# andimarafioti/faster-qwen3-tts

Measured on AMD Instinct MI355X. Metric: real-time factor (audio s / wall s), Qwen3-TTS-12Hz-0.6B voice-clone streaming chunk_size=8; p50 TTFA in ttfa_ms_p50, higher is better.
Workload: dtype bf16

## Files before the change

faster-qwen3-tts_amd/csrc/fq3_api.hip:

```cpp
#define FQ3_SKINNY_EXTERN
#include "fq3_ctx.h"
#include "sampler.cuh"
#include "sampler_wave.cuh"
#include "skinny_gemm.cuh"

#include <cstdio>
#include <cstdlib>
#include <cstring>
#include <map>
#include <string>
#include <type_traits>
#include <vector>

using namespace fq3;

static thread_local std::string g_err;
static int fail(int code, const std::string& m) { g_err = m; return code; }
int fq3_fail_(int code, const std::string& m) { return fail(code, m); }
#define HIPCHK(x) do { hipError_t e_ = (x); if (e_ != hipSuccess) return fail(FQ3_EHIP, std::string(#x) + ": " + hipGetErrorString(e_)); } while (0)

extern "C" const char* fq3_last_error(void) { return g_err.c_str(); }
extern "C" void fq3_set_error_(const char* msg) { g_err = msg ? msg : ""; }
extern "C" int fq3_abi_version(void) { return FQ3_ABI_VERSION; }

// ... 184 lines not shown
    const int Vm = std::max(t.vocab, p.vocab);
    const int G = cfg->num_code_groups;
    const int frames = cfg->max_frames > 0 ? cfg->max_frames : 4096;
    c->cfg.max_frames = frames;
    if ((r = dmalloc(c, &c->h, (size_t)Hm * c->esz))) return r;
    if ((r = dmalloc(c, &c->h2, (size_t)Hm * c->esz))) return r;
    if ((r = dmalloc(c, &c->qkv2, (size_t)qkvm * c->esz))) return r;
    if ((r = dmalloc(c, &c->attn_out, (size_t)qkvm * c->esz))) return r;
    if ((r = dmalloc(c, &c->attn_out2, (size_t)qkvm * c->esz))) return r;
    if ((r = dmalloc(c, &c->act2, (size_t)Im * c->esz))) return r;
    if ((r = dmalloc(c, &c->pred_x2, (size_t)p.hidden * c->esz))) return r;
    if ((r = dmalloc(c, &c->xin, (size_t)Hm * c->esz))) return r;
    if ((r = dmalloc(c, &c->tmp_hidden, (size_t)Hm * c->esz))) return r;
    if ((r = dmalloc(c, &c->qkv, (size_t)qkvm * c->esz))) return r;
    if ((r = dmalloc(c, &c->act, (size_t)Im * c->esz))) return r;
    if ((r = dmalloc(c, &c->logits, (size_t)Vm * c->esz))) return r;
    if ((r = dmalloc(c, &c->past_hidden, (size_t)t.hidden * c->esz))) return r;
    if ((r = dmalloc(c, &c->ph_hold, (size_t)t.hidden * c->esz))) return r;
    if ((r = dmalloc(c, &c->pred_in, (size_t)2 * t.hidden * c->esz))) return r;
    if ((r = dmalloc(c, &c->pred_next, (size_t)t.hidden * c->esz))) return r;
    if ((r = dmalloc(c, &c->pred_x, (size_t)p.hidden * c->esz))) return r;
    if ((r = dmalloc(c, &c->plogits, (size_t)(G - 1) * p.vocab * c->esz))) return r;
    const int maxkv = std::max(t.n_kv_heads, p.n_kv_heads);
    c->part_stride = (size_t)maxkv * kMaxWorkers * 4 * kPartStride;
    if ((r = dmalloc(c, (void**)&c->part, 2 * c->part_stride * sizeof(float)))) return r;
    if ((r = dmalloc(c, (void**)&c->rope_now, 2 * 64 * sizeof(float)))) return r;
    if ((r = dmalloc(c, (void**)&c->seen_api, kMaxVocab))) return r;
    if ((r = dmalloc(c, (void**)&c->st, sizeof(DecodeState)))) return r;
    if ((r = dmalloc(c, (void**)&c->seen, kMaxVocab))) return r;
    if ((r = dmalloc(c, (void**)&c->codes, (size_t)(frames + 1) * G * sizeof(int)))) return r;
    if ((r = dmalloc(c, (void**)&c->ids64, (size_t)64 * sizeof(int64_t)))) return r;
    if ((r = dmalloc(c, (void**)&c->d_pemb, (size_t)64 * sizeof(void*)))) return r;
    HIPCHK(hipStreamCreateWithFlags(&c->cap_stream, hipStreamNonBlocking));
    return FQ3_OK;
}

extern "C" int fq3_set_option(fq3_ctx* c, const char* key, int value) {
    if (!c || !key) return fail(FQ3_EINVAL, "null argument");
    const std::string k(key);
    if (k == "weight_nt") c->opt_nt = value;
    else if (k == "pred_m2") c->opt_m2 = value;
    else if (k == "pred_attn") c->opt_pred_attn = value;
    else if (k == "rows_per_wave_max") c->opt_rmax = value;
    else if (k == "prefill_mode") c->prefill_mode = value;
    else if (k == "flash_prefill") c->opt_flash_prefill = value;
    else if (k == "flash_small") c->opt_flash_small = value;
    else if (k == "swiglu_tile") c->opt_swiglu_tile = value;
    else if (k == "packed_weights") c->opt_packed = value;
    else if (k == "skinny_gemm") c->opt_no_skinny = !value;
    else return fail(FQ3_EINVAL, "unknown option: " + k);
    fq3_graph_reset(c);
    return FQ3_OK;
}

extern "C" int fq3_graph_reset(fq3_ctx* c) {
    if (!c) return fail(FQ3_EINVAL, "null ctx");
    if (c->exec) { (void)hipGraphExecDestroy(c->exec); c->exec = nullptr; }
    if (c->graph) { (void)hipGraphDestroy(c->graph); c->graph = nullptr; }
    return FQ3_OK;
}

namespace {
struct PackedEntry { void* p; int refs; int N, K; };
std::mutex g_packed_mu;
std::map<std::pair<const void*, int>, PackedEntry> g_packed;
}
// ... 30 lines not shown
}
static int packed_acquire_all(fq3_ctx* c) {
    if (c->cfg.dtype != FQ3_BF16) return FQ3_OK;
    auto take = [&](const void* W, int N, int K, int kind) -> int {
        const int r = fq3_packed_acquire_(W, N, K, kind);
        if (r == FQ3_OK) c->packed_refs.emplace_back(W, kind);
        return r == FQ3_EUNSUPPORTED ? FQ3_OK : r;
    };
    auto stack = [&](const std::vector<fq3_layer_weights>& L, const fq3_stack_dims& d) -> int {
        const int qd = d.n_heads * kHeadDim, kvd = d.n_kv_heads * kHeadDim;
        for (const fq3_layer_weights& l : L) {
            if (int r = take(l.qkv, qd + 2 * kvd, d.hidden, 0)) return r;
            if (int r = take(l.o, d.hidden, qd, 0)) return r;
            if (int r = take(l.gate_up, 2 * d.inter, d.hidden, 1)) return r;
            if (int r = take(l.gate_up, 2 * d.inter, d.hidden, 0)) return r;
            if (int r = take(l.down, d.hidden, d.inter, 0)) return r;
        }
        return FQ3_OK;
    };
    if (int r = stack(c->tl, c->cfg.talker)) return r;
    if (int r = stack(c->pl, c->cfg.predictor)) return r;
    for (const fq3_layer_weights& l : c->tl) if (int r = take(l.gate_up, 2 * c->cfg.talker.inter, c->cfg.talker.hidden, 2)) return r;
    if (int r = take(c->wt.codec_head, c->cfg.talker.vocab, c->cfg.talker.hidden, 0)) return r;
    for (const void* h : c->lmh) if (int r = take(h, c->cfg.predictor.vocab, c->cfg.predictor.hidden, 0)) return r;
    return FQ3_OK;
}

extern "C" int fq3_ctx_destroy(fq3_ctx* c) {
    if (!c) return FQ3_OK;
    (void)hipDeviceSynchronize();
    fq3_graph_reset(c);
    packed_release_all(c);
    if (c->cap_stream) (void)hipStreamDestroy(c->cap_stream);
    if (fq3_kv_pool* p = c->tk.pool) {
        (void)fq3_kv_release(c, 0);
        bool last;
        { std::lock_guard<std::mutex> lk(p->mu); last = --p->users == 0; }
        if (p->is_private && last) pool_free_(p);
    }
    for (void* p : c->allocs) (void)hipFree(p);
    delete c;
    return FQ3_OK;
}

extern "C" int fq3_bind_weights(fq3_ctx* c, const fq3_weight_table* w) {
    if (!c || !w) return fail(FQ3_EINVAL, "null argument");
    const int G = c->cfg.num_code_groups;
    if (!w->talker_layers || !w->predictor_layers || !w->codec_embedding || !w->codec_head || !w->talker_final_norm ||
        !w->predictor_final_norm || !w->predictor_embeddings || !w->lm_heads || !w->talker_cos || !w->talker_sin ||
        !w->pred_cos || !w->pred_sin)
        return fail(FQ3_EINVAL, "weight table has null entries");
    if (c->cfg.has_projection && !w->proj_w) return fail(FQ3_EINVAL, "has_projection set but proj_w is null");
    if (w->talker_rope_len < c->cfg.max_seq_len || w->pred_rope_len < G + 1)
        return fail(FQ3_EINVAL, "rope tables shorter than the caches");
    c->wt = *w;
    c->tl.assign(w->talker_layers, w->talker_layers + c->cfg.talker.n_layers);
    c->pl.assign(w->predictor_layers, w->predictor_layers + c->cfg.predictor.n_layers);
    c->pemb.assign(w->predictor_embeddings, w->predictor_embeddings + (G - 1));
    c->lmh.assign(w->lm_heads, w->lm_heads + (G - 1));
    for (auto& l : c->tl) if (!l.qkv || !l.o || !l.gate_up || !l.down || !l.input_norm || !l.post_norm || !l.q_norm || !l.k_norm)
        return fail(FQ3_EINVAL, "talker layer has null weights");
    for (auto& l : c->pl) if (!l.qkv || !l.o || !l.gate_up || !l.down || !l.input_norm || !l.post_norm || !l.q_norm || !l.k_norm)
        return fail(FQ3_EINVAL, "predictor layer has null weights");
    HIPCHK(hipMemcpy(c->d_pemb, c->pemb.data(), (G - 1) * sizeof(void*), hipMemcpyHostToDevice));
    (void)hipDeviceSynchronize();
    packed_release_all(c);
// ... 585 lines not shown
    tf->forced = forced; tf->decisions = decisions;
}

extern "C" int fq3_decode_begin(fq3_ctx* c, const fq3_decode_params* p, void* stream) {
    NEED_BOUND(c);
    if (!p || !p->past_hidden || !p->tts_pad_embed) return fail(FQ3_EINVAL, "null argument");
    if (p->trailing_len > 0 && !p->trailing_text) return fail(FQ3_EINVAL, "trailing_text");
    if (p->talker.do_sample && (!p->talker_noise || p->noise_frames <= 0)) return fail(FQ3_EINVAL, "talker sampling needs a noise ring");
    if (c->pred_sampling.do_sample && (!p->pred_noise || p->noise_frames <= 0)) return fail(FQ3_EINVAL, "predictor sampling needs a noise ring");
    if (p->talker.do_sample && !(p->talker.temperature > 0.f)) return fail(FQ3_EINVAL, "temperature must be > 0");
    if (p->max_new_tokens > c->cfg.max_frames) return fail(FQ3_EINVAL, "max_new_tokens exceeds the context's max_frames");
    if (p->prefill_len <= 0 || p->prefill_len > c->cfg.max_seq_len) return fail(FQ3_EINVAL, "prefill_len");
    if (p->first_token < 0 || p->first_token >= c->cfg.talker.vocab) return fail(FQ3_EINVAL, "first_token outside the codec vocabulary");
    if (p->gen_step < 0 || p->min_new_tokens < 0 || p->max_new_tokens < 0) return fail(FQ3_EINVAL, "negative counters");
    const bool wave = p->talker.top_p >= 1.0f;
    if (wave != c->talker_wave) { fq3_graph_reset(c); c->talker_wave = wave; }
    hipStream_t s = (hipStream_t)stream;
    if (int r = fq3_kv_ensure_(c, p->prefill_len + p->max_new_tokens + 1, s)) return r;
    DecodeState h{};
    h.token = p->first_token; h.frame = 0; h.pos = p->prefill_len; h.gen_step = p->gen_step; h.done = 0; h.text_open = 0;
    h.min_new = p->min_new_tokens; h.max_new = p->max_new_tokens; h.trailing_len = p->trailing_len;
    h.noise_frames = p->noise_frames > 0 ? p->noise_frames : 1;
    h.eos_id = c->cfg.codec_eos_token_id; h.max_seq = c->cfg.max_seq_len;
    h.n_pad = c->n_pad; h.rope_delta = c->rope_delta;
    h.sup_lo = c->cfg.talker.vocab - 1024 > 0 ? c->cfg.talker.vocab - 1024 : 0; h.sup_hi = c->cfg.talker.vocab;
    h.t_temperature = p->talker.temperature; h.t_top_k = p->talker.top_k; h.t_top_p = p->talker.top_p;
    h.t_do_sample = p->talker.do_sample; h.t_rep_penalty = p->talker.repetition_penalty;
    h.p_temperature = c->pred_sampling.temperature; h.p_top_k = c->pred_sampling.top_k; h.p_top_p = c->pred_sampling.top_p;
    h.p_do_sample = c->pred_sampling.do_sample;
    h.trailing_text = p->trailing_text; h.tts_pad = p->tts_pad_embed; h.talker_noise = p->talker_noise; h.pred_noise = p->pred_noise;
    hipLaunchKernelGGL(decode_arm_kernel, dim3(1), dim3(256), 0, s, c->st, h, c->seen, (int)kMaxVocab,
                       (uint32_t*)c->past_hidden, (const uint32_t*)p->past_hidden, (int)((size_t)c->cfg.talker.hidden * c->esz / 4));
    LAUNCH_CHECK();
    c->armed = true; c->tt_open = false; c->tt_session = false; c->tt_rows = 0; c->tt_cap = 0;
    c->begin_trailing = p->trailing_text; c->begin_trailing_len = p->trailing_len > 0 ? p->trailing_len : 0;
    return FQ3_OK;
}

__global__ void decode_cancel_kernel(DecodeState* st) { st->done = 1; }
extern "C" int fq3_decode_cancel(fq3_ctx* c, void* stream) {
    if (!c) return fail(FQ3_EINVAL, "null ctx");
    hipLaunchKernelGGL(decode_cancel_kernel, dim3(1), dim3(1), 0, (hipStream_t)stream, c->st);
    LAUNCH_CHECK();
    return FQ3_OK;
}

extern "C" int fq3_decode_set_forced(fq3_ctx* c, const int32_t* forced_codes, int32_t* decisions, void* stream) {
    NEED_BOUND(c);
    if (!c->tf) {
        if (!forced_codes && !decisions) return FQ3_OK;
        if (int r = dmalloc(c, (void**)&c->tf, sizeof(TeacherForcing))) return r;
        fq3_graph_reset(c);
    }
    hipLaunchKernelGGL(decode_set_forced_kernel, dim3(1), dim3(1), 0, (hipStream_t)stream, c->tf, forced_codes, decisions);
    LAUNCH_CHECK();
    return FQ3_OK;
}

template <typename T>
static int enqueue_frame_t(fq3_ctx* c, hipStream_t s) {
    const fq3_stack_dims& t = c->cfg.talker;
    const int G = c->cfg.num_code_groups, H = t.hidden;
    DecodeState* st = c->st;
    hipLaunchKernelGGL((frame_begin_kernel<T>), dim3(1), dim3(256), 0, s, st, (const T*)c->wt.codec_embedding,
                       (const T*)c->past_hidden, (T*)c->ph_hold, (T*)c->pred_in, c->codes, c->seen, H, G);
    if (int r = predictor_passes_t<T>(c, st, c->pred_in, nullptr, nullptr, nullptr, s)) return r;
// ... 16 lines not shown
    return c->cfg.dtype == FQ3_BF16 ? enqueue_frame_t<bf16_t>(c, s) : enqueue_frame_t<float>(c, s);
}

extern "C" int fq3_graph_capture(fq3_ctx* c, void* stream) {
    NEED_BOUND(c);
    if (c->exec) return FQ3_OK;
    (void)stream;
    hipStream_t cs = c->cap_stream;
    HIPCHK(hipStreamBeginCapture(cs, hipStreamCaptureModeRelaxed));
    int r = enqueue_frame(c, cs);
    hipGraph_t g = nullptr;
    hipError_t e = hipStreamEndCapture(cs, &g);
    if (r) { if (g) (void)hipGraphDestroy(g); return r; }
    if (e != hipSuccess) return fail(FQ3_EHIP, std::string("hipStreamEndCapture: ") + hipGetErrorString(e));
    c->graph = g;
    HIPCHK(hipGraphInstantiate(&c->exec, c->graph, nullptr, nullptr, 0));
    return FQ3_OK;
}

extern "C" int fq3_decode_frames(fq3_ctx* c, int n_frames, void* stream) {
    NEED_BOUND(c);
    hipStream_t s = (hipStream_t)stream;
    for (int i = 0; i < n_frames; ++i) {
        if (c->exec) { HIPCHK(hipGraphLaunch(c->exec, s)); }
        else if (int r = enqueue_frame(c, s)) return r;
    }
    LAUNCH_CHECK();
    return FQ3_OK;
}

extern "C" int fq3_decode_poll(fq3_ctx* c, int* n_frames_total, int* done, void* stream) {
    if (!c) return fail(FQ3_EINVAL, "null ctx");
    hipStream_t s = (hipStream_t)stream;
    DecodeState h;
    HIPCHK(hipMemcpyAsync(&h, c->st, sizeof h, hipMemcpyDeviceToHost, s));
    HIPCHK(hipStreamSynchronize(s));
    if (n_frames_total) *n_frames_total = h.frame;
    if (done) *done = h.done == 2 ? 2 : (h.done || h.token == h.eos_id);
    return FQ3_OK;
}

__global__ void codes_to_i64_kernel(const int* src, int64_t* dst, int n) {
    const int i = blockIdx.x * blockDim.x + threadIdx.x;
    if (i < n) dst[i] = src[i];
}

extern "C" int fq3_decode_codes(fq3_ctx* c, int from, int count, int64_t* out, void* stream) {
    if (!c || !out) return fail(FQ3_EINVAL, "null argument");
    if (from < 0 || count < 0 || from + count > c->cfg.max_frames) return fail(FQ3_EINVAL, "range");
    const int G = c->cfg.num_code_groups, n = count * G;
    if (n == 0) return FQ3_OK;
    hipLaunchKernelGGL(codes_to_i64_kernel, dim3((n + 255) / 256), dim3(256), 0, (hipStream_t)stream,
                       c->codes + (size_t)from * G, out, n);
    LAUNCH_CHECK();
    return FQ3_OK;
}
```

faster-qwen3-tts_amd/csrc/fq3_ctx.h:

```cpp
#pragma once
#include "../../include/fq3hip.h"
#include "decode_kernels.cuh"
#include <hip/hip_runtime.h>
#include <mutex>
#include <string>
#include <utility>
#include <vector>

struct fq3_kv_pool {
    int dtype = 0, esz = 2, n_layers = 0, n_kv = 0, n_blocks = 0;
    size_t blk_elems = 0;
    std::vector<void*> k, v;
    std::vector<int> free_list;
    std::mutex mu;
    int in_use_high = 0;
    int users = 0;
    bool is_private = false;
};

struct StackBufs {
    std::vector<void*> k, v;
    int max_seq = 0, workers = 1;
    fq3_kv_pool* pool = nullptr;
    int* d_table = nullptr;
    std::vector<int> blocks;
    int max_blocks = 0;
};

struct fq3_ctx {
    fq3_config cfg{};
    int esz = 2;
    std::vector<fq3_layer_weights> tl, pl;
    fq3_weight_table wt{};
    std::vector<const void*> pemb, lmh;
    const void** d_pemb = nullptr;
    bool bound = false;
    StackBufs tk, pk;
    void *h = nullptr, *xin = nullptr, *qkv = nullptr, *act = nullptr, *logits = nullptr, *past_hidden = nullptr;
    void *pred_in = nullptr, *pred_x = nullptr, *pred_next = nullptr, *plogits = nullptr, *tmp_hidden = nullptr;
    void *attn_out = nullptr, *attn_out2 = nullptr;
    void *h2 = nullptr, *qkv2 = nullptr, *act2 = nullptr, *pred_x2 = nullptr;
    size_t part_stride = 0;
    float* part = nullptr;
    float* rope_now = nullptr;
    unsigned char* seen_api = nullptr;
    fq3::DecodeState* st = nullptr;
    fq3::TeacherForcing* tf = nullptr;
    unsigned char* seen = nullptr;
    int* codes = nullptr;
    int64_t* ids64 = nullptr;
    int n_pad = 0, rope_delta = 0;
    int opt_nt = 1;
    int opt_m2 = 1;
    int opt_pred_attn = 1;
    int opt_rmax = 2;
    int opt_flash_prefill = 1;
    int opt_flash_small = 1;
    int opt_swiglu_tile = 1;
    int opt_packed = 1;
    std::vector<std::pair<const void*, int>> packed_refs;
    int opt_no_skinny = 0;
    int prefill_mode = 0;
    bool talker_wave = true;
    fq3_sampling pred_sampling{0.9f, 50, 1.0f, 1, 1.0f};
    hipGraph_t graph = nullptr;
    hipGraphExec_t exec = nullptr;
    hipStream_t cap_stream = nullptr;
    std::vector<void*> allocs;
    fq3_prompt_weights pw{};
    bool pw_bound = false;
    void *pw_x = nullptr, *pw_h = nullptr;
    int pw_cap = 0;
    void* ph_hold = nullptr;
    void *tt_tab = nullptr, *tt_x = nullptr, *tt_h = nullptr;
    int tt_alloc = 0;
    int tt_cap = 0, tt_rows = 0;
    bool tt_open = false, tt_session = false;
    bool armed = false;
    const void* begin_trailing = nullptr; int begin_trailing_len = 0;
    void *pf_x = nullptr, *pf_xn = nullptr, *pf_qkv = nullptr, *pf_att = nullptr, *pf_gu = nullptr, *pf_act = nullptr, *pf_ws = nullptr;
};


const void* fq3_packed_find_(const void* W, int kind);
int fq3_packed_acquire_(const void* W, int N, int K, int kind);
void fq3_packed_release_(const void* W, int kind);

int fq3_fail_(int code, const std::string& m);
int fq3_kv_ensure_(fq3_ctx* c, int n_pos, hipStream_t s);
int fq3_prefill_reserve_(fq3_ctx* c);
int fq3_prefill_mfma_(fq3_ctx* c, const void* embeds, int L, int n_pad, void* out_logits, void* out_hidden, hipStream_t s);
int fq3_prefill_batch_mfma_(fq3_ctx* const* cs, int n, const void* const* embeds, const int* L, const int* n_pad, void* const* out_logits,
                            void* const* out_hidden, hipStream_t s);
int fq3_codec_head_launch_(fq3_ctx* c, const void* hidden, void* out_logits, hipStream_t s);
int fq3_dmalloc_(fq3_ctx* c, void** p, size_t bytes);
void fq3_text_project_launch_(fq3_ctx* c, const int64_t* ids, int n, void* x, void* h, void* out, hipStream_t s);
```

faster-qwen3-tts_amd/fq3hip/_lib.py:

```python
from __future__ import annotations

import ctypes as C
import os

import torch

_HERE = os.path.dirname(os.path.abspath(__file__))
LIB_PATH = os.path.join(os.path.dirname(_HERE), "lib", "libfq3hip.so")

FQ3_BF16, FQ3_F32, FQ3_BF16X2 = 0, 1, 2
FQ3_OK, FQ3_EINVAL, FQ3_EHIP, FQ3_ESTATE, FQ3_ETOOLONG, FQ3_EUNSUPPORTED, FQ3_ENOMEM = 0, -1, -2, -3, -4, -5, -6

vp = C.c_void_p
i32 = C.c_int32


class StackDims(C.Structure):
    _fields_ = [("hidden", i32), ("inter", i32), ("n_layers", i32), ("n_heads", i32), ("n_kv_heads", i32),
                ("head_dim", i32), ("vocab", i32), ("rms_eps", C.c_float)]


class Config(C.Structure):
    _fields_ = [("dtype", i32), ("talker", StackDims), ("predictor", StackDims), ("num_code_groups", i32),
                ("max_seq_len", i32), ("codec_eos_token_id", i32), ("has_projection", i32), ("max_frames", i32)]
# ... 54 lines not shown
    "fq3_ctx_create": (C.c_int, [C.POINTER(Config), C.POINTER(vp)]),
    "fq3_ctx_destroy": (C.c_int, [vp]),
    "fq3_kv_pool_create": (C.c_int, [C.POINTER(Config), C.c_int, C.POINTER(vp)]),
    "fq3_kv_pool_destroy": (C.c_int, [vp]),
    "fq3_kv_pool_stats": (C.c_int, [vp, C.POINTER(C.c_int), C.POINTER(C.c_int), C.POINTER(C.c_int), C.POINTER(C.c_int64)]),
    "fq3_ctx_create_pooled": (C.c_int, [C.POINTER(Config), vp, C.POINTER(vp)]),
    "fq3_kv_reserve": (C.c_int, [vp, C.c_int, vp]),
    "fq3_kv_release": (C.c_int, [vp, C.c_int]),
    "fq3_kv_blocks": (C.c_int, [vp]),
    "fq3_bind_weights": (C.c_int, [vp, C.POINTER(WeightTable)]),
    "fq3_set_option": (C.c_int, [vp, C.c_char_p, C.c_int]),
    "fq3_kv_import": (C.c_int, [vp, C.c_int, vp, vp, C.c_int, vp]),
    "fq3_kv_export": (C.c_int, [vp, C.c_int, vp, vp, C.c_int, vp]),
    "fq3_kv_adopt": (C.c_int, [vp, vp, C.c_int, vp]),
    "fq3_set_generation_state": (C.c_int, [vp, C.c_int, C.c_int]),
    "fq3_talker_step": (C.c_int, [vp, vp, C.c_int, vp, vp]),
    "fq3_prefill": (C.c_int, [vp, vp, C.c_int, C.c_int, vp, vp, vp]),
    "fq3_prefill_reserve": (C.c_int, [vp]),
    "fq3_prefill_batch": (C.c_int, [C.POINTER(vp), C.c_int, C.POINTER(vp), C.POINTER(C.c_int), C.POINTER(C.c_int), C.POINTER(vp),
                                    C.POINTER(vp), vp]),
    "fq3_set_prefill_mode": (C.c_int, [vp, C.c_int]),
    "fq3_codec_head": (C.c_int, [vp, vp, vp, vp]),
    "fq3_set_predictor_sampling": (C.c_int, [vp, C.POINTER(Sampling)]),
    "fq3_predictor_loop": (C.c_int, [vp, vp, vp, vp, vp, vp]),
    "fq3_sample": (C.c_int, [vp, vp, C.c_int, C.POINTER(Sampling), vp, C.c_int, C.c_int, C.c_int, C.c_int,
                             C.c_int, vp, vp, vp]),
    "fq3_apply_repetition_penalty": (C.c_int, [vp, vp, C.c_int, vp, C.c_int, C.c_float, vp]),
    "fq3_decode_begin": (C.c_int, [vp, C.POINTER(DecodeParams), vp]),
    "fq3_decode_cancel": (C.c_int, [vp, vp]),
    "fq3_decode_set_forced": (C.c_int, [vp, vp, vp, vp]),
    "fq3_decode_frames": (C.c_int, [vp, C.c_int, vp]),
    "fq3_decode_poll": (C.c_int, [vp, C.POINTER(C.c_int), C.POINTER(C.c_int), vp]),
    "fq3_decode_codes": (C.c_int, [vp, C.c_int, C.c_int, vp, vp]),
    "fq3_graph_capture": (C.c_int, [vp, vp]),
    "fq3_graph_reset": (C.c_int, [vp]),
    "fq3_bind_prompt_weights": (C.c_int, [vp, C.POINTER(PromptWeights)]),
    "fq3_text_project": (C.c_int, [vp, vp, C.c_int, vp, vp]),
    "fq3_decode_text_open": (C.c_int, [vp, C.c_int, vp]),
    "fq3_decode_text_append": (C.c_int, [vp, vp, C.c_int, C.c_int, vp]),
    "fq3_decode_text_rows": (C.c_int, [vp, C.POINTER(C.c_int), C.POINTER(C.c_int)]),
    "fq3_decode_text_read": (C.c_int, [vp, C.c_int, C.c_int, vp, vp]),
    "fq3_prompt_rows": (C.c_int, [vp, vp, C.c_int, vp, C.c_int, vp, C.c_int, vp, vp, vp]),
    "fq3_batch_create": (C.c_int, [C.POINTER(vp), C.c_int, C.POINTER(vp)]),
    "fq3_batch_destroy": (C.c_int, [vp]),
    "fq3_batch_size": (C.c_int, [vp]),
    "fq3_batch_frames": (C.c_int, [vp, C.c_int, vp]),
    "fq3_batch_graph_capture": (C.c_int, [vp, vp]),
    "fq3_batch_graph_reset": (C.c_int, [vp]),
    "fq3_batch_set_option": (C.c_int, [vp, C.c_char_p, C.c_int]),
    "fq3_batch_set_group_streams": (C.c_int, [vp, C.POINTER(vp), C.c_int]),
    "fq3_batch_poll_async": (C.c_int, [vp, C.c_int, vp]),
    "fq3_batch_poll_wait": (C.c_int, [vp, C.c_int, C.POINTER(C.c_int), C.POINTER(C.c_int)]),
    "fq3_batch_text_append": (C.c_int, [vp, C.c_int, C.POINTER(C.c_int32), C.POINTER(C.c_int32), C.POINTER(C.c_int32), vp, vp]),
    "fq3_codec_create": (C.c_int, [C.POINTER(CodecConfig), C.POINTER(vp)]),
    "fq3_codec_destroy": (C.c_int, [vp]),
    "fq3_codec_set_option": (C.c_int, [vp, C.c_char_p, C.c_int]),
    "fq3_codec_bind": (C.c_int, [vp, C.c_char_p, vp, C.c_int64]),
    "fq3_codec_finalize": (C.c_int, [vp, vp]),
    "fq3_codec_num_samples": (C.c_int64, [vp, C.c_int]),
    "fq3_codec_decode": (C.c_int, [vp, vp, C.c_int, vp, vp]),
    "fq3_codec_decode_tail": (C.c_int, [vp, vp, C.c_int, C.c_int64, vp, vp]),
    "fq3_codec_decode_batch": (C.c_int, [vp, vp, C.c_int, C.c_int, C.c_int64, vp, vp]),
    "fq3_codec_prefix_create": (C.c_int, [vp, vp, C.c_int, C.POINTER(vp), vp]),
    "fq3_codec_prefix_destroy": (C.c_int, [vp]),
    "fq3_codec_prefix_frames": (C.c_int, [vp]),
    "fq3_codec_decode_batch_prefix": (C.c_int, [vp, C.POINTER(vp), vp, C.c_int, C.c_int, C.c_int64, vp, vp]),
# ... 45 lines not shown
```

faster-qwen3-tts_amd/fq3hip/engine.py:

```python
from __future__ import annotations

import ctypes as C
import threading
from typing import Dict, Optional

import torch

from . import _lib as L
from .config import TTSConfig, StackConfig

Weights = Dict[str, torch.Tensor]
_CAPTURE_LOCK = threading.Lock()


def _ptr(t: Optional[torch.Tensor]) -> Optional[int]:
    return None if t is None else t.data_ptr()


def rope_tables(head_dim: int, theta: float, n_pos: int, dtype: torch.dtype):
    inv = 1.0 / (theta ** (torch.arange(0, head_dim, 2, dtype=torch.float) / head_dim))
    ang = torch.arange(n_pos, dtype=torch.float32)[:, None] * inv[None, :]
    return ang.cos().to(dtype).float().contiguous(), ang.sin().to(dtype).float().contiguous()


# ... 343 lines not shown
        tl = trailing_text.shape[-2] if trailing_text is not None and trailing_text.numel() else 0
        if tl:
            self._chk(trailing_text, tl * H, "trailing_text")
        p = L.DecodeParams()
        p.talker = L.Sampling(float(temperature), int(top_k), float(top_p), int(bool(do_sample)), float(repetition_penalty))
        p.min_new_tokens, p.max_new_tokens = int(min_new_tokens), int(max_new_tokens)
        p.prefill_len, p.gen_step, p.first_token = int(prefill_len), int(gen_step), int(first_token)
        p.past_hidden, p.trailing_text, p.trailing_len = past_hidden.data_ptr(), _ptr(trailing_text) if tl else None, tl
        p.tts_pad_embed = tts_pad_embed.data_ptr()
        p.talker_noise, p.pred_noise, p.noise_frames = _ptr(talker_noise), _ptr(pred_noise), int(noise_frames)
        self._loop_keep = (past_hidden, trailing_text, tts_pad_embed, talker_noise, pred_noise)
        L.check(self.lib.fq3_decode_begin(self.ctx, C.byref(p), self._stream()))

    def graph_capture(self):
        with _CAPTURE_LOCK:
            L.check(self.lib.fq3_graph_capture(self.ctx, self._stream()))

    def graph_reset(self):
        L.check(self.lib.fq3_graph_reset(self.ctx))

    def decode_frames(self, n: int):
        L.check(self.lib.fq3_decode_frames(self.ctx, int(n), self._stream()))

    def decode_poll(self):
        n, d = C.c_int(0), C.c_int(0)
        L.check(self.lib.fq3_decode_poll(self.ctx, C.byref(n), C.byref(d), self._stream()))
        return n.value, bool(d.value)

    def decode_poll_state(self):
        n, d = C.c_int(0), C.c_int(0)
        L.check(self.lib.fq3_decode_poll(self.ctx, C.byref(n), C.byref(d), self._stream()))
        return n.value, int(d.value)

    def decode_text_open(self, capacity_rows: int):
        L.check(self.lib.fq3_decode_text_open(self.ctx, int(capacity_rows), self._stream()))

    def decode_text_append(self, ids, final: bool = False):
        if isinstance(ids, torch.Tensor):
            t = ids.reshape(-1).to(device=self.device, dtype=torch.long).contiguous()
        else:
            t = torch.tensor([int(i) for i in ids], dtype=torch.long, device=self.device)
        n = int(t.numel())
        L.check(self.lib.fq3_decode_text_append(self.ctx, t.data_ptr() if n else None, n, int(bool(final)), self._stream()))
        self._text_ids_keep = t

    def decode_text_rows(self):
        n, c = C.c_int(0), C.c_int(0)
        L.check(self.lib.fq3_decode_text_rows(self.ctx, C.byref(n), C.byref(c)))
        return n.value, bool(c.value)

    def decode_text_read(self, start: int = 0, count: Optional[int] = None) -> torch.Tensor:
        if count is None:
            count = self.decode_text_rows()[0] - int(start)
        out = self.new(int(count), self.cfg.talker.hidden_size)
        L.check(self.lib.fq3_decode_text_read(self.ctx, int(start), int(count), out.data_ptr(), self._stream()))
        return out

    def decode_codes(self, start: int, count: int) -> torch.Tensor:
        out = torch.empty(count, self.cfg.num_code_groups, dtype=torch.long, device=self.device)
        if count:
            L.check(self.lib.fq3_decode_codes(self.ctx, int(start), int(count), out.data_ptr(), self._stream()))
        return out

    def close(self):
        if getattr(self, "ctx", None) and self.ctx.value:
            self.lib.fq3_ctx_destroy(self.ctx)
# ... 87 lines not shown
```

faster-qwen3-tts_amd/fq3hip/generate.py:

```python
from __future__ import annotations

import time
from typing import Optional, Tuple

import torch

from .predictor_graph import PredictorGraph
from .talker_graph import TalkerGraph

NOISE_RING = 64


def _refill(engine, talker_noise, pred_noise):
    if talker_noise is not None:
        talker_noise.exponential_(1)
    if pred_noise is not None:
        pred_noise.exponential_(1)


def _n_pad_of(attention_mask) -> int:
    if attention_mask is None:
        return 0
    known = noted_n_pad(attention_mask)
    return known if known is not None else int((attention_mask[0] == 0).sum())


def noted_n_pad(attention_mask):
    note = getattr(attention_mask, "fq3_n_pad", None)
    if not (isinstance(note, tuple) and len(note) == 2):
        return None
    if note[1] is None:
        return int(note[0])
    if attention_mask.is_inference() or note[1] != attention_mask._version:
        return None
    return int(note[0])


def _prefill_first_token(eng, talker_input_embeds, attention_mask, config, min_new_tokens, temperature, top_k, top_p, do_sample):
    dt, dev = eng.dtype, eng.device
    eos_id = config.codec_eos_token_id
    V = config.vocab_size
    n_pad = _n_pad_of(attention_mask)
    x = talker_input_embeds[0].to(device=dev, dtype=dt).contiguous()
# ... 58 lines not shown
    max_frames = min(int(max_new_tokens), eng.max_frames)
    eng.decode_begin(first_token=int(token), prefill_len=prefill_len, gen_step=gen_step, past_hidden=hidden,
                     trailing_text=tth, tts_pad_embed=tpe, temperature=temperature, top_k=top_k, top_p=top_p,
                     do_sample=do_sample, repetition_penalty=repetition_penalty, min_new_tokens=min_new_tokens,
                     max_new_tokens=max_frames, talker_noise=tn, pred_noise=pn, noise_frames=NOISE_RING)
    if use_graph:
        eng.graph_capture()
    else:
        eng.graph_reset()
    return eng, tn, pn, max_frames


def _prefill_and_arm(talker, talker_input_embeds, attention_mask, trailing_text_hiddens, tts_pad_embed, config,
                     predictor_graph, talker_graph, max_new_tokens, min_new_tokens, temperature, top_k, top_p,
                     do_sample, repetition_penalty, use_graph):
    token, hidden, n_rows, n_pad = _prefill_first_token(talker_graph.engine, talker_input_embeds, attention_mask, config,
                                                        min_new_tokens, temperature, top_k, top_p, do_sample)
    return _arm_decode(talker, config, token, hidden, n_rows, attention_mask, trailing_text_hiddens, tts_pad_embed, predictor_graph,
                       talker_graph, max_new_tokens, min_new_tokens, temperature, top_k, top_p, do_sample, repetition_penalty,
                       use_graph, n_pad=n_pad)


def run_frames(eng, tn, pn, issued: int, count: int):
    while count > 0:
        if issued % NOISE_RING == 0:
            _refill(eng, tn, pn)
        k = min(count, NOISE_RING - issued % NOISE_RING)
        eng.decode_frames(k)
        issued += k
        count -= k
    return issued


@torch.inference_mode()
def fast_generate(talker, talker_input_embeds: torch.Tensor, attention_mask: torch.Tensor,
                  trailing_text_hiddens: torch.Tensor, tts_pad_embed: torch.Tensor, config,
                  predictor_graph: PredictorGraph, talker_graph: TalkerGraph, max_new_tokens: int = 2048,
                  min_new_tokens: int = 2, temperature: float = 0.9, top_k: int = 50, top_p: float = 1.0,
                  do_sample: bool = True, repetition_penalty: float = 1.05,
                  subtalker_dosample: Optional[bool] = None, subtalker_top_k: Optional[int] = None,
                  subtalker_top_p: Optional[float] = None, subtalker_temperature: Optional[float] = None,
                  parity_mode: bool = False, poll_every: int = 8) -> Tuple[Optional[torch.Tensor], dict]:
    t_start = time.time()
    eng, tn, pn, max_frames = _prefill_and_arm(
        talker, talker_input_embeds, attention_mask, trailing_text_hiddens, tts_pad_embed, config, predictor_graph,
        talker_graph, max_new_tokens, min_new_tokens, temperature, top_k, top_p, do_sample, repetition_penalty,
        use_graph=not parity_mode)
    torch.cuda.current_stream(eng.device).synchronize()
    t_prefill = time.time() - t_start
    t_decode_start = time.time()
    issued, n, done = 0, 0, False
    while not done and issued < max_frames:
        issued = run_frames(eng, tn, pn, issued, min(poll_every, max_frames - issued))
        n, done = eng.decode_poll()
    codes = eng.decode_codes(0, n) if n > 0 else None
    torch.cuda.current_stream(eng.device).synchronize()
    t_decode = time.time() - t_decode_start
    timing = {
        "prefill_ms": t_prefill * 1000,
        "decode_s": t_decode,
        "steps": n,
        "ms_per_step": (t_decode / n * 1000) if n > 0 else 0,
        "steps_per_s": (n / t_decode) if t_decode > 0 else 0,
    }
    return codes, timing
```

faster-qwen3-tts_amd/fq3hip/streaming.py:

```python
from __future__ import annotations

import time
from typing import Generator, Tuple

import torch

from .generate import _prefill_and_arm, run_frames
from .predictor_graph import PredictorGraph
from .talker_graph import TalkerGraph


@torch.inference_mode()
def fast_generate_streaming(talker, talker_input_embeds: torch.Tensor, attention_mask: torch.Tensor,
                            trailing_text_hiddens: torch.Tensor, tts_pad_embed: torch.Tensor, config,
                            predictor_graph: PredictorGraph, talker_graph: TalkerGraph, max_new_tokens: int = 2048,
                            min_new_tokens: int = 2, temperature: float = 0.9, top_k: int = 50, top_p: float = 1.0,
                            do_sample: bool = True, repetition_penalty: float = 1.05, chunk_size: int = 12,
                            use_graph: bool = True) -> Generator[Tuple[torch.Tensor, dict], None, None]:
    t_start = time.time()
    eng, tn, pn, max_frames = _prefill_and_arm(
        talker, talker_input_embeds, attention_mask, trailing_text_hiddens, tts_pad_embed, config, predictor_graph,
        talker_graph, max_new_tokens, min_new_tokens, temperature, top_k, top_p, do_sample, repetition_penalty,
        use_graph=use_graph)
    torch.cuda.current_stream(eng.device).synchronize()
    t_prefill = time.time() - t_start
    issued, emitted, chunk_count, done = 0, 0, 0, False
    chunk_start = time.time()
    issued = run_frames(eng, tn, pn, issued, min(chunk_size, max_frames))
    while True:
        n, done = eng.decode_poll()
        new = n - emitted
        if new <= 0:
            break
        chunk = eng.decode_codes(emitted, new)
        ready = torch.cuda.Event()
        ready.record(torch.cuda.current_stream(eng.device))
        emitted = n
        is_final = new < chunk_size
        more = (not done) and (not is_final) and issued < max_frames
        if more:
            issued = run_frames(eng, tn, pn, issued, min(chunk_size, max_frames - issued))
        yield chunk, {
            "chunk_index": chunk_count,
            "chunk_steps": new,
            "prefill_ms": t_prefill * 1000 if chunk_count == 0 else 0,
            "decode_ms": (time.time() - chunk_start) * 1000,
            "total_steps_so_far": emitted,
            "is_final": is_final,
            "codes_ready_event": ready,
        }
        chunk_count += 1
        chunk_start = time.time()
        if not more:
            break


def parity_generate_streaming(talker, talker_input_embeds, attention_mask, trailing_text_hiddens, tts_pad_embed, config,
                              max_new_tokens: int = 2048, min_new_tokens: int = 2, temperature: float = 0.9,
                              top_k: int = 50, top_p: float = 1.0, do_sample: bool = True,
                              repetition_penalty: float = 1.05, chunk_size: int = 12, predictor_graph=None,
                              talker_graph=None):
    if predictor_graph is None or talker_graph is None:
        raise ValueError("parity_generate_streaming needs the graph objects of the HIP context")
    return fast_generate_streaming(talker, talker_input_embeds, attention_mask, trailing_text_hiddens, tts_pad_embed,
                                   config, predictor_graph, talker_graph, max_new_tokens=max_new_tokens,
                                   min_new_tokens=min_new_tokens, temperature=temperature, top_k=top_k, top_p=top_p,
                                   do_sample=do_sample, repetition_penalty=repetition_penalty, chunk_size=chunk_size,
                                   use_graph=False)
```

include/fq3hip.h:

```cpp
#ifndef FQ3HIP_H
#define FQ3HIP_H

#include <stdint.h>

#ifdef __cplusplus
extern "C" {
#endif

#define FQ3_ABI_VERSION 5

enum { FQ3_BF16 = 0, FQ3_F32 = 1,
       FQ3_BF16X2 = 2 };
enum { FQ3_OK = 0, FQ3_EINVAL = -1, FQ3_EHIP = -2, FQ3_ESTATE = -3, FQ3_ETOOLONG = -4, FQ3_EUNSUPPORTED = -5, FQ3_ENOMEM = -6 };

typedef struct fq3_stack_dims {
    int32_t hidden, inter, n_layers, n_heads, n_kv_heads, head_dim, vocab;
    float rms_eps;
} fq3_stack_dims;

typedef struct fq3_config {
    int32_t dtype;
    fq3_stack_dims talker;
    fq3_stack_dims predictor;
    int32_t num_code_groups;
// ... 85 lines not shown
                       void* out_logits, void* stream);


int fq3_sample(fq3_ctx* ctx, const void* logits, int V, const fq3_sampling* s, const int64_t* history,
               int n_hist, int sup_lo, int sup_hi, int keep_id, int suppress_eos, const void* noise,
               int64_t* out_token, void* stream);

int fq3_apply_repetition_penalty(fq3_ctx* ctx, void* logits, int V, const int64_t* history, int n_hist, float penalty,
                                 void* stream);


typedef struct fq3_decode_params {
    fq3_sampling talker;
    int32_t min_new_tokens;
    int32_t max_new_tokens;
    int32_t prefill_len;
    int32_t gen_step;
    int32_t first_token;
    const void* past_hidden;
    const void* trailing_text;
    int32_t trailing_len;
    const void* tts_pad_embed;
    const void* talker_noise;
    const void* pred_noise;
    int32_t noise_frames;
} fq3_decode_params;

int fq3_decode_begin(fq3_ctx* ctx, const fq3_decode_params* p, void* stream);
int fq3_decode_cancel(fq3_ctx* ctx, void* stream);
int fq3_decode_set_forced(fq3_ctx* ctx, const int32_t* forced_codes, int32_t* decisions, void* stream);
int fq3_decode_frames(fq3_ctx* ctx, int n_frames, void* stream);
int fq3_decode_poll(fq3_ctx* ctx, int* n_frames_total, int* done, void* stream);
int fq3_decode_codes(fq3_ctx* ctx, int from, int count, int64_t* out_codes_dev, void* stream);
int fq3_graph_capture(fq3_ctx* ctx, void* stream);
int fq3_graph_reset(fq3_ctx* ctx);

typedef struct fq3_prompt_weights {
    const void* text_embedding;
    const void* fc1_w;
    const void* fc1_b;
    const void* fc2_w;
    const void* fc2_b;
    int32_t text_vocab, text_hidden;
} fq3_prompt_weights;
int fq3_bind_prompt_weights(fq3_ctx* ctx, const fq3_prompt_weights* w);
int fq3_text_project(fq3_ctx* ctx, const int64_t* ids, int n, void* out, void* stream);
int fq3_prompt_rows(fq3_ctx* ctx, const void* text_rows, int n_text, const int32_t* prog, int n_rows,
                    const int64_t* ref_codes, int n_ref, const void* spk_embed, void* out, void* stream);

int fq3_decode_text_open(fq3_ctx* ctx, int capacity_rows, void* stream);
int fq3_decode_text_append(fq3_ctx* ctx, const int64_t* ids, int n, int final, void* stream);
int fq3_decode_text_rows(const fq3_ctx* ctx, int* n_rows, int* closed);
int fq3_decode_text_read(fq3_ctx* ctx, int from, int count, void* out, void* stream);

typedef struct fq3_batch fq3_batch;
int fq3_batch_create(fq3_ctx* const* lanes, int n_lanes, fq3_batch** out);
int fq3_batch_destroy(fq3_batch* b);
int fq3_batch_size(const fq3_batch* b);
int fq3_batch_frames(fq3_batch* b, int n_frames, void* stream);
int fq3_batch_graph_capture(fq3_batch* b, void* stream);
int fq3_batch_graph_reset(fq3_batch* b);
int fq3_batch_poll_async(fq3_batch* b, int slot, void* stream);
int fq3_batch_poll_wait(fq3_batch* b, int slot, int* n_frames_total, int* done);
int fq3_batch_text_append(fq3_batch* b, int n_items, const int32_t* lane, const int32_t* count, const int32_t* final_,
                          const int64_t* ids, void* stream);
int fq3_batch_set_option(fq3_batch* b, const char* key, int value);
// ... 55 lines not shown
```

Before: 37.15.

## Queue async decode polls and run frames ahead of chunk marker

Adds an asynchronous poll API: a small kernel snapshots decode state and copies the chunk's codes, then writes the status into pinned host memory tracked by an event per slot. The streaming and non-streaming loops now issue a few frames beyond each chunk marker before waiting on the poll, so the GPU stays busy while the host reads status and yields chunks. The goal is to remove the idle GPU bubble caused by a blocking stream synchronize and a separate codes copy each chunk. The cost is extra frames of speculative work after EOS and more complex slot and event bookkeeping.

```diff
diff --git a/faster-qwen3-tts_amd/csrc/fq3_api.hip b/faster-qwen3-tts_amd/csrc/fq3_api.hip
--- a/faster-qwen3-tts_amd/csrc/fq3_api.hip
+++ b/faster-qwen3-tts_amd/csrc/fq3_api.hip
@@ -240,6 +240,9 @@
     if ((r = dmalloc(c, (void**)&c->ids64, (size_t)64 * sizeof(int64_t)))) return r;
     if ((r = dmalloc(c, (void**)&c->d_pemb, (size_t)64 * sizeof(void*)))) return r;
     HIPCHK(hipStreamCreateWithFlags(&c->cap_stream, hipStreamNonBlocking));
+    if ((r = dmalloc(c, (void**)&c->poll_dev, (size_t)kDecodePollSlots * 2 * sizeof(int)))) return r;
+    HIPCHK(hipHostMalloc((void**)&c->poll_host, (size_t)kDecodePollSlots * 2 * sizeof(int) + sizeof(DecodeState), hipHostMallocDefault));
+    for (int i = 0; i < kDecodePollSlots; ++i) HIPCHK(hipEventCreateWithFlags(&c->poll_ev[i], hipEventDisableTiming));
     return FQ3_OK;
 }
 
@@ -336,6 +339,8 @@
     fq3_graph_reset(c);
     packed_release_all(c);
     if (c->cap_stream) (void)hipStreamDestroy(c->cap_stream);
+    for (hipEvent_t e : c->poll_ev) if (e) (void)hipEventDestroy(e);
+    if (c->poll_host) (void)hipHostFree(c->poll_host);
     if (fq3_kv_pool* p = c->tk.pool) {
         (void)fq3_kv_release(c, 0);
         bool last;
@@ -987,6 +992,7 @@
     hipLaunchKernelGGL(decode_arm_kernel, dim3(1), dim3(256), 0, s, c->st, h, c->seen, (int)kMaxVocab,
                        (uint32_t*)c->past_hidden, (const uint32_t*)p->past_hidden, (int)((size_t)c->cfg.talker.hidden * c->esz / 4));
     LAUNCH_CHECK();
+    for (bool& a : c->poll_armed) a = false;
     c->armed = true; c->tt_open = false; c->tt_session = false; c->tt_rows = 0; c->tt_cap = 0;
     c->begin_trailing = p->trailing_text; c->begin_trailing_len = p->trailing_len > 0 ? p->trailing_len : 0;
     return FQ3_OK;
@@ -1069,11 +1075,50 @@
 extern "C" int fq3_decode_poll(fq3_ctx* c, int* n_frames_total, int* done, void* stream) {
     if (!c) return fail(FQ3_EINVAL, "null ctx");
     hipStream_t s = (hipStream_t)stream;
-    DecodeState h;
-    HIPCHK(hipMemcpyAsync(&h, c->st, sizeof h, hipMemcpyDeviceToHost, s));
+    DecodeState* h = (DecodeState*)(c->poll_host + kDecodePollSlots * 2);
+    HIPCHK(hipMemcpyAsync(h, c->st, sizeof *h, hipMemcpyDeviceToHost, s));
     HIPCHK(hipStreamSynchronize(s));
-    if (n_frames_total) *n_frames_total = h.frame;
-    if (done) *done = h.done == 2 ? 2 : (h.done || h.token == h.eos_id);
+    if (n_frames_total) *n_frames_total = h->frame;
+    if (done) *done = h->done == 2 ? 2 : (h->done || h->token == h->eos_id);
+    return FQ3_OK;
+}
+
+__global__ void decode_poll_kernel(const DecodeState* st, int* slot, const int* src, int64_t* dst, int n) {
+    const int i = blockIdx.x * blockDim.x + threadIdx.x;
+    if (i == 0) {
+        slot[0] = st->frame;
+        slot[1] = st->done == 2 ? 2 : ((st->done || st->token == st->eos_id) ? 1 : 0);
+    }
+    if (i < n) dst[i] = src[i];
+}
+
+extern "C" int fq3_decode_poll_async(fq3_ctx* c, int slot, int from_frame, int count, int64_t* codes_out, void* stream) {
+    if (!c) return fail(FQ3_EINVAL, "null ctx");
+    if (slot < 0 || slot >= kDecodePollSlots) return fail(FQ3_EINVAL, "poll slot must be 0..3");
+    if (from_frame < 0 || count < 0 || from_frame + count > c->cfg.max_frames) return fail(FQ3_EINVAL, "range");
+    if (count > 0 && !codes_out) return fail(FQ3_EINVAL, "null argument");
+    if (c->poll_armed[slot]) return fail(FQ3_ESTATE, "a poll is still queued in this slot");
+    hipStream_t s = (hipStream_t)stream;
+    const int G = c->cfg.num_code_groups, n = count * G;
+    int* d = c->poll_dev + 2 * slot;
+    hipLaunchKernelGGL(decode_poll_kernel, dim3(n > 0 ? (n + 255) / 256 : 1), dim3(256), 0, s, c->st, d,
+                       c->codes + (size_t)from_frame * G, codes_out, n);
+    LAUNCH_CHECK();
+    HIPCHK(hipMemcpyAsync(c->poll_host + 2 * slot, d, 2 * sizeof(int), hipMemcpyDeviceToHost, s));
+    HIPCHK(hipEventRecord(c->poll_ev[slot], s));
+    c->poll_armed[slot] = true;
+    return FQ3_OK;
+}
+
+extern "C" int fq3_decode_poll_wait(fq3_ctx* c, int slot, int* n_frames_total, int* done) {
+    if (!c) return fail(FQ3_EINVAL, "null ctx");
+    if (slot < 0 || slot >= kDecodePollSlots) return fail(FQ3_EINVAL, "poll slot must be 0..3");
+    if (!c->poll_armed[slot]) return fail(FQ3_ESTATE, "no poll was queued in this slot");
+    HIPCHK(hipEventSynchronize(c->poll_ev[slot]));
+    c->poll_armed[slot] = false;
+    const int* h = c->poll_host + 2 * slot;
+    if (n_frames_total) *n_frames_total = h[0];
+    if (done) *done = h[1];
     return FQ3_OK;
 }
 
diff --git a/faster-qwen3-tts_amd/csrc/fq3_ctx.h b/faster-qwen3-tts_amd/csrc/fq3_ctx.h
--- a/faster-qwen3-tts_amd/csrc/fq3_ctx.h
+++ b/faster-qwen3-tts_amd/csrc/fq3_ctx.h
@@ -26,6 +26,8 @@
     std::vector<int> blocks;
     int max_blocks = 0;
 };
+
+constexpr int kDecodePollSlots = 4;
 
 struct fq3_ctx {
     fq3_config cfg{};
@@ -77,6 +79,10 @@
     int tt_cap = 0, tt_rows = 0;
     bool tt_open = false, tt_session = false;
     bool armed = false;
+    int* poll_dev = nullptr;
+    int* poll_host = nullptr;
+    hipEvent_t poll_ev[kDecodePollSlots] = {};
+    bool poll_armed[kDecodePollSlots] = {};
     const void* begin_trailing = nullptr; int begin_trailing_len = 0;
     void *pf_x = nullptr, *pf_xn = nullptr, *pf_qkv = nullptr, *pf_att = nullptr, *pf_gu = nullptr, *pf_act = nullptr, *pf_ws = nullptr;
 };
diff --git a/faster-qwen3-tts_amd/fq3hip/_lib.py b/faster-qwen3-tts_amd/fq3hip/_lib.py
--- a/faster-qwen3-tts_amd/fq3hip/_lib.py
+++ b/faster-qwen3-tts_amd/fq3hip/_lib.py
@@ -110,6 +110,8 @@
     "fq3_decode_frames": (C.c_int, [vp, C.c_int, vp]),
     "fq3_decode_poll": (C.c_int, [vp, C.POINTER(C.c_int), C.POINTER(C.c_int), vp]),
     "fq3_decode_codes": (C.c_int, [vp, C.c_int, C.c_int, vp, vp]),
+    "fq3_decode_poll_async": (C.c_int, [vp, C.c_int, C.c_int, C.c_int, vp, vp]),
+    "fq3_decode_poll_wait": (C.c_int, [vp, C.c_int, C.POINTER(C.c_int), C.POINTER(C.c_int)]),
     "fq3_graph_capture": (C.c_int, [vp, vp]),
     "fq3_graph_reset": (C.c_int, [vp]),
     "fq3_bind_prompt_weights": (C.c_int, [vp, C.POINTER(PromptWeights)]),
diff --git a/faster-qwen3-tts_amd/fq3hip/engine.py b/faster-qwen3-tts_amd/fq3hip/engine.py
--- a/faster-qwen3-tts_amd/fq3hip/engine.py
+++ b/faster-qwen3-tts_amd/fq3hip/engine.py
@@ -399,6 +399,17 @@
         L.check(self.lib.fq3_decode_poll(self.ctx, C.byref(n), C.byref(d), self._stream()))
         return n.value, int(d.value)
 
+    def decode_poll_async(self, slot: int, start: int, count: int) -> torch.Tensor:
+        out = torch.empty(int(count), self.cfg.num_code_groups, dtype=torch.long, device=self.device)
+        L.check(self.lib.fq3_decode_poll_async(self.ctx, int(slot), int(start), int(count), out.data_ptr() if count else None,
+                                               self._stream()))
+        return out
+
+    def decode_poll_wait(self, slot: int):
+        n, d = C.c_int(0), C.c_int(0)
+        L.check(self.lib.fq3_decode_poll_wait(self.ctx, int(slot), C.byref(n), C.byref(d)))
+        return n.value, bool(d.value)
+
     def decode_text_open(self, capacity_rows: int):
         L.check(self.lib.fq3_decode_text_open(self.ctx, int(capacity_rows), self._stream()))
 
diff --git a/faster-qwen3-tts_amd/fq3hip/generate.py b/faster-qwen3-tts_amd/fq3hip/generate.py
--- a/faster-qwen3-tts_amd/fq3hip/generate.py
+++ b/faster-qwen3-tts_amd/fq3hip/generate.py
@@ -9,6 +9,7 @@
 from .talker_graph import TalkerGraph
 
 NOISE_RING = 64
+RUN_AHEAD = 2
 
 
 def _refill(engine, talker_noise, pred_noise):
@@ -133,6 +134,32 @@
     return issued
 
 
+def plan_issue(issued: int, marker: int, chunk: int, max_frames: int, run_ahead: int, ring: int = NOISE_RING) -> Tuple[int, int]:
+    marker = min(marker, max_frames)
+    to_marker = max(0, marker - issued)
+    start = issued + to_marker
+    end = min(marker + min(run_ahead, chunk), max_frames)
+    if marker % ring == 0:
+        end = marker
+    else:
+        end = min(end, (marker // ring + 1) * ring)
+    return to_marker, max(0, end - start)
+
+
+def poll_queue(eng, slot: int, start: int, count: int):
+    if hasattr(eng, "decode_poll_async"):
+        return eng.decode_poll_async(slot, start, count)
+    return None
+
+
+def poll_read(eng, slot: int, queued):
+    return eng.decode_poll() if queued is None else eng.decode_poll_wait(slot)
+
+
+def run_ahead_of(eng) -> int:
+    return RUN_AHEAD if hasattr(eng, "decode_poll_async") else 0
+
+
 @torch.inference_mode()
 def fast_generate(talker, talker_input_embeds: torch.Tensor, attention_mask: torch.Tensor,
                   trailing_text_hiddens: torch.Tensor, tts_pad_embed: torch.Tensor, config,
@@ -150,10 +177,16 @@
     torch.cuda.current_stream(eng.device).synchronize()
     t_prefill = time.time() - t_start
     t_decode_start = time.time()
-    issued, n, done = 0, 0, False
-    while not done and issued < max_frames:
-        issued = run_frames(eng, tn, pn, issued, min(poll_every, max_frames - issued))
-        n, done = eng.decode_poll()
+    issued, marker, n, done, k = 0, 0, 0, False, 0
+    ahead = run_ahead_of(eng)
+    while not done and marker < max_frames:
+        marker = min(marker + poll_every, max_frames)
+        to_marker, more = plan_issue(issued, marker, poll_every, max_frames, ahead)
+        issued = run_frames(eng, tn, pn, issued, to_marker)
+        queued = poll_queue(eng, k % 2, 0, 0)
+        issued = run_frames(eng, tn, pn, issued, more)
+        n, done = poll_read(eng, k % 2, queued)
+        k += 1
     codes = eng.decode_codes(0, n) if n > 0 else None
     torch.cuda.current_stream(eng.device).synchronize()
     t_decode = time.time() - t_decode_start
diff --git a/faster-qwen3-tts_amd/fq3hip/streaming.py b/faster-qwen3-tts_amd/fq3hip/streaming.py
--- a/faster-qwen3-tts_amd/fq3hip/streaming.py
+++ b/faster-qwen3-tts_amd/fq3hip/streaming.py
@@ -5,7 +5,7 @@
 
 import torch
 
-from .generate import _prefill_and_arm, run_frames
+from .generate import _prefill_and_arm, plan_issue, poll_queue, poll_read, run_ahead_of, run_frames
 from .predictor_graph import PredictorGraph
 from .talker_graph import TalkerGraph
 
@@ -25,21 +25,35 @@
     torch.cuda.current_stream(eng.device).synchronize()
     t_prefill = time.time() - t_start
     issued, emitted, chunk_count, done = 0, 0, 0, False
+    ahead = run_ahead_of(eng)
+    stream = torch.cuda.current_stream(eng.device)
+
+    def issue_chunk(issued, marker, slot):
+        to_marker, more = plan_issue(issued, marker, chunk_size, max_frames, ahead)
+        issued = run_frames(eng, tn, pn, issued, to_marker)
+        queued = poll_queue(eng, slot, emitted, marker - emitted)
+        ready = torch.cuda.Event()
+        ready.record(stream)
+        return run_frames(eng, tn, pn, issued, more), queued, ready
+
     chunk_start = time.time()
-    issued = run_frames(eng, tn, pn, issued, min(chunk_size, max_frames))
+    marker = min(chunk_size, max_frames)
+    issued, queued, ready = issue_chunk(issued, marker, 0)
     while True:
-        n, done = eng.decode_poll()
+        n, done = poll_read(eng, chunk_count % 2, queued)
         new = n - emitted
         if new <= 0:
             break
-        chunk = eng.decode_codes(emitted, new)
-        ready = torch.cuda.Event()
-        ready.record(torch.cuda.current_stream(eng.device))
+        chunk = queued[:new] if queued is not None else eng.decode_codes(emitted, new)
+        if queued is None:
+            ready = torch.cuda.Event()
+            ready.record(stream)
         emitted = n
         is_final = new < chunk_size
-        more = (not done) and (not is_final) and issued < max_frames
+        more = (not done) and (not is_final) and marker < max_frames
         if more:
-            issued = run_frames(eng, tn, pn, issued, min(chunk_size, max_frames - issued))
+            marker = min(marker + chunk_size, max_frames)
+            issued, queued, next_ready = issue_chunk(issued, marker, (chunk_count + 1) % 2)
         yield chunk, {
             "chunk_index": chunk_count,
             "chunk_steps": new,
@@ -53,6 +67,7 @@
         chunk_start = time.time()
         if not more:
             break
+        ready = next_ready
 
 
 def parity_generate_streaming(talker, talker_input_embeds, attention_mask, trailing_text_hiddens, tts_pad_embed, config,
diff --git a/include/fq3hip.h b/include/fq3hip.h
--- a/include/fq3hip.h
+++ b/include/fq3hip.h
@@ -141,6 +141,8 @@
 int fq3_decode_frames(fq3_ctx* ctx, int n_frames, void* stream);
 int fq3_decode_poll(fq3_ctx* ctx, int* n_frames_total, int* done, void* stream);
 int fq3_decode_codes(fq3_ctx* ctx, int from, int count, int64_t* out_codes_dev, void* stream);
+int fq3_decode_poll_async(fq3_ctx* ctx, int slot, int from_frame, int count, int64_t* codes_out, void* stream);
+int fq3_decode_poll_wait(fq3_ctx* ctx, int slot, int* n_frames_total, int* done);
 int fq3_graph_capture(fq3_ctx* ctx, void* stream);
 int fq3_graph_reset(fq3_ctx* ctx);
 
```

Result: no change. 37.31 (median of 2 runs) (+0.4%).
